# jp-schneider/awesome

Hardware: AMD Instinct MI355X
Metric: INR-fits/sec (256x256 grid, convexity prior) (higher is better)
Workload: dtype f32; 1 GPU; 1 x 256x256 synthetic convex blob per GPU, ConvexNextNet(h=130,L=1), SE(sigmoid) mean, Adam lr 2e-3, clamp, E=2000 full-batch steps (BASELINE configs[1]); images_per_gpu=1, grid=256x256, epochs_per_fit=2000, parallelism=dp1 (independent fits)

## Files before the change

### awesome_amd/csrc/icnn_step.h

```cpp
#pragma once
#include <hip/hip_runtime.h>
#include <stdint.h>
#include <math.h>

#include <type_traits>

#include "inrfit.h"

typedef float f32x4 __attribute__((ext_vector_type(4)));
typedef float f32x2 __attribute__((ext_vector_type(2)));

#define MFMA16(a, b, c) __builtin_amdgcn_mfma_f32_16x16x4f32((a), (b), (c), 0, 0, 0)
__device__ __forceinline__ float relu0(float x) { return __int_as_float(max(__float_as_int(x), 0)); }
constexpr float INV_2PI = 0.15915494309189535f;
__device__ __forceinline__ float hw_sin(float x) { return __builtin_amdgcn_sinf(__builtin_amdgcn_fractf(x * INV_2PI)); }
__device__ __forceinline__ float hw_cos(float x) { return __builtin_amdgcn_cosf(__builtin_amdgcn_fractf(x * INV_2PI)); }
template <int ACT>
__device__ __forceinline__ float act0_f(float pre, float omega) {
    if constexpr (ACT == INR_ACT_COS) return hw_cos(pre);
    else if constexpr (ACT == INR_ACT_SIN) return hw_sin(omega * pre);
    else return relu0(pre);
}
template <int ACT>
__device__ __forceinline__ float dact0_f(float pre, float omega) {
// ... 78 lines not shown
                        : SL_WO + (j - P_WO);
    }
};

struct ImgMap {
    int H, C, L, HM, S, PT, floats;
    int off_sc, off_wine, off_win, off_bin, off_floor, off_wo;
    int off_wct[2], off_w[2];
    int ext[4];
    int p_bin, p_wo, p_bo, p_so, P;
    int p_w[2], p_b[2], p_s[2];
    int sl_tile;
    int sl_cols;
    int KG, kg_magic;
    int identity;
};

__device__ __forceinline__ int slab_param_of_col(const ImgMap& m, int col) {
    if (m.identity) return col < m.sl_cols ? col : -1;
    const int H = m.H, HM = m.HM, C = m.C, KG = m.KG, kgm = m.kg_magic, T = m.sl_tile, two = m.L > 1;
    const int e0 = m.ext[0], e1 = m.ext[1], e2 = m.ext[2], e3 = m.ext[3], pwo = m.p_wo, ncols = m.sl_cols;
    const int tl = (two && col >= T) ? 1 : 0, ct = col - tl * T;
    const int pw = tl ? m.p_w[1] : m.p_w[0], pb = tl ? m.p_b[1] : m.p_b[0], ps = tl ? m.p_s[1] : m.p_s[0];
    const int r = ct & 3, lane = (ct >> 2) & 63, tb = ct >> 8;
    const int rt = (tb * kgm) >> 16, b = tb - rt * KG;
    const int o = 16 * rt + 4 * (lane >> 4) + r, pos = 16 * b + (lane & 15);
    int tile = -1;
    tile = (pos == e3 && C > 2) ? ps + o * C + 2 : tile;
    tile = (pos == e2 && C > 1) ? ps + o * C + 1 : tile;
    tile = pos == e1 ? ps + o * C : tile;
    tile = pos == e0 ? pb + o : tile;
    tile = pos < H ? pw + o * H + pos : tile;
    const int HR = H - HM, LS = HR * (H + 1 + C), NT = two ? 2 * T : T;
    const int c = col - NT, c1 = c - m.p_w[0];
    const int rl = (two && c1 >= LS) ? 1 : 0, cl = c1 - rl * LS;
    const int qw = rl ? m.p_w[1] : m.p_w[0], qb = rl ? m.p_b[1] : m.p_b[0], qs = rl ? m.p_s[1] : m.p_s[0];
    const int c2 = cl - HR * H, c3 = c2 - HR;
    int rest = qs + HM * C + c3;
    rest = c3 < 0 ? qb + HM + c2 : rest;
    rest = c2 < 0 ? qw + HM * H + cl : rest;
    const int ct2 = c1 - (two ? 2 * LS : LS);
    rest = ct2 >= 0 ? pwo + ct2 : rest;
    rest = c1 < 0 ? c : rest;
    const int res = col < NT ? tile : rest;
    return col < ncols ? res : -1;
}

__device__ __forceinline__ int image_slots(const ImgMap& m, int j, int (&slot)[2]) {
    if (j < m.p_bin) {
        const int i = j / m.C, c = j - i * m.C;
        slot[0] = m.off_wine + c * m.PT + i;
        if (i >= m.HM) {
            slot[1] = m.off_win + c * 16 + (i - m.HM);
            return 2;
        }
        return 1;
    }
    if (j < m.p_w[0]) {
        const int i = j - m.p_bin;
        slot[0] = m.off_wine + m.C * m.PT + i;
        if (i >= m.HM) {
            slot[1] = m.off_bin + (i - m.HM);
            return 2;
        }
        return 1;
    }
    for (int k = 0; k < m.L; ++k) {
        if (j < m.p_b[k]) {
            const int q = j - m.p_w[k];
            const int o = q / m.H, i = q - o * m.H;
            slot[0] = m.off_w[k] + o * m.S + i;
            if (i >= m.HM) {
                slot[1] = m.off_wct[k] + (i - m.HM) * m.PT + o;
                return 2;
            }
            return 1;
        }
        if (j < m.p_s[k]) {
            slot[0] = m.off_w[k] + (j - m.p_b[k]) * m.S + m.ext[0];
            return 1;
        }
        if (j < m.p_s[k] + m.H * m.C) {
            const int q = j - m.p_s[k];
            const int o = q / m.C, c = q - o * m.C;
            slot[0] = m.off_w[k] + o * m.S + m.ext[1 + c];
            return 1;
        }
    }
    if (j < m.p_bo) {
        slot[0] = m.off_wo + (j - m.p_wo);
        return 1;
    }
    slot[0] = m.off_sc + (j - m.p_bo);
    return 1;
}

struct StepArgs {
    const float* wimg;
    const float* targets;
    const float* coef;
    float* slabs;
    float* loss_part;
    float* logits;
    float* dcoords;
    InrGridDesc grid;
    long long N;
    int n_images, wgs, PS, loss_kind;
    float act_omega;
    const float* seg;
    float c_align;
    int data_count;
    int use_noneclass;
    float noneclass;
    int align_soft;
    int align_begin;
};

template <int CTRL>
__device__ __forceinline__ float dpp_f(float v) {
    return __int_as_float(__builtin_amdgcn_update_dpp(0, __float_as_int(v), CTRL, 0xF, 0xF, true));
}
__device__ __forceinline__ float bce_log(float x) {
    const float l = logf(x);
    return l < -100.f ? -100.f : l;
}

__device__ __forceinline__ void align_term(const float* __restrict__ seg, float c_align, int soft, float pr, float& l, float& dy) {
    const float s = *seg;
    const float d = pr - (soft ? s : (s > 0.5f ? 1.f : 0.f));
    const float cd = c_align * d;
    l = fmaf(cd, d, l);
    dy = fmaf(2.f * cd, pr * (1.f - pr), dy);
}

__device__ __forceinline__ float sum_over_points(float v) {
    v += dpp_f<0xB1>(v);
    v += dpp_f<0x4E>(v);
    v += dpp_f<0x141>(v);
    v += dpp_f<0x140>(v);
    return v;
}
__device__ __forceinline__ float sum_over_groups(float v) {
    {
        const auto r = __builtin_amdgcn_permlane16_swap(__float_as_uint(v), __float_as_uint(v), false, false);
        v = __uint_as_float(r[0]) + __uint_as_float(r[1]);
    }
    {
        const auto r = __builtin_amdgcn_permlane32_swap(__float_as_uint(v), __float_as_uint(v), false, false);
        v = __uint_as_float(r[0]) + __uint_as_float(r[1]);
    }
    return v;
}

#ifndef INR_SCHED_HINTS
#define INR_SCHED_HINTS 1
#endif
#if INR_SCHED_HINTS
#define SGB(mask, n) __builtin_amdgcn_sched_group_barrier((mask), (n), 0)
#else
#define SGB(mask, n)
#endif
#ifndef INR_BWD_B128
#define INR_BWD_B128 0
#endif
#ifndef INR_STAGE_Z0_EARLY
#define INR_STAGE_Z0_EARLY 1
#endif
#ifndef INR_PROLOGUE_EARLY
#define INR_PROLOGUE_EARLY 1
#endif
#ifndef INR_SLAB_NT
#define INR_SLAB_NT 1
#endif
#ifndef INR_TILES_SPREAD
#define INR_TILES_SPREAD 1
#endif
#ifndef INR_MFMA_ORDER
#define INR_MFMA_ORDER 1
#endif
#if INR_MFMA_ORDER
#define MFMA_STEP_FENCE() __builtin_amdgcn_sched_barrier(0x7F6)
#define OPERAND_FENCE() __builtin_amdgcn_sched_barrier(0x676)
#else
#define MFMA_STEP_FENCE()
#define OPERAND_FENCE()
#endif

#ifndef INR_STAMPS
#define INR_STAMPS 0
#endif
#if INR_STAMPS
__device__ unsigned long long g_stamps[16];
__device__ unsigned long long g_wgtimes[1024][4];
__device__ unsigned long long g_wgfirst[1024];
#define STAMP(k)                                                                                   \
    do {                                                                                           \
        __builtin_amdgcn_sched_barrier(0);                                                         \
        unsigned long long t_;                                                                     \
        asm volatile("s_memtime %0\n\ts_waitcnt lgkmcnt(0)" : "=s"(t_)::"memory");                 \
        __builtin_amdgcn_sched_barrier(0);                                                         \
        st_sum[k] += t_ - st_prev;                                                                 \
        st_prev = t_;                                                                              \
    } while (0)
#else
#define STAMP(k)
#endif

template <int FLOATS>
__device__ __forceinline__ f32x4 image_to_lds_issue(const float* __restrict__ gimg, float* smem, const int tid, const int lane, const int wave) {
    constexpr int PIECES = FLOATS / 256, TAIL4 = (FLOATS - 256 * PIECES) / 4;
    static_assert(FLOATS % 4 == 0 && TAIL4 <= 256, "the tail is one float4 per thread at most");
    f32x4 tail = f32x4{0.f, 0.f, 0.f, 0.f};
    if (tid < TAIL4) tail = ((const f32x4*)gimg)[64 * PIECES + tid];
#pragma unroll
    for (int k = 0; k < (PIECES + 3) / 4; ++k) {
        const int pc = wave + 4 * k;
        if (pc < PIECES)
            __builtin_amdgcn_global_load_lds((const __attribute__((address_space(1))) void*)(gimg + pc * 256 + lane * 4),
                                             (__attribute__((address_space(3))) void*)(smem + pc * 256), 16, 0, 0);
    }
    return tail;
}
template <int FLOATS>
__device__ __forceinline__ void image_tail_to_lds(float* smem, const int tid, const f32x4 tail) {
    constexpr int PIECES = FLOATS / 256, TAIL4 = (FLOATS - 256 * PIECES) / 4;
    if (tid < TAIL4) ((f32x4*)smem)[64 * PIECES + tid] = tail;
}

template <int H, int C, bool TRAIN, bool DX = false, int ACT0 = INR_ACT_RELU>
__global__ __launch_bounds__(WG_THREADS, 1) void icnn_step_kernel(const StepArgs a) {
    static_assert(!DX || TRAIN, "coordinate gradients are a by-product of the backward pass");
    static_assert(!DX || ACT0 == INR_ACT_RELU, "the coordinate-gradient kernels are built for relu networks only");
    using G = Cfg<H, C>;
    constexpr int TM = G::TM, KG = G::KG, HM = G::HM, HR = G::HR, S = G::S, PT = G::PT, RPW = G::RPW, NEXT = G::NEXT;
    constexpr bool B128 = INR_BWD_B128 && (TM % 4 == 0);
    auto bcol = [](int t, int l) { return B128 ? 64 * (t >> 2) + 4 * l + (t & 3) : 16 * t + l; };
    constexpr int HRA = HR > 0 ? HR : 1;
    static_assert(TM % RPW == 0, "row tiles must split evenly over the waves that own rows");
    extern __shared__ __attribute__((aligned(16))) float smem[];
    float* const Wimg = smem + G::OFF_W;
    float* const WcT = smem + G::OFF_WCT;
    float* const WinE = smem + G::OFF_WINE;
    float* const WinT = smem + G::OFF_WIN;
    float* const binT = smem + G::OFF_BIN;
    float* const floorT = smem + G::OFF_FLOOR;
    float* const woT = smem + G::OFF_WO;
    float* const stA = smem + G::OFF_STA;
    float* const stB = smem + G::OFF_STB;

#if INR_STAMPS
    const unsigned long long rt_entry = __builtin_amdgcn_s_memrealtime();
#endif
    const int tid = threadIdx.x;
    const int lane = tid & 63;
    const int wave = __builtin_amdgcn_readfirstlane(tid >> 6);
    const int l15 = lane & 15, g = lane >> 4;
    const int img = blockIdx.x / a.wgs;
    const int wg = blockIdx.x - img * a.wgs;
    const long long N = a.N;

    const float* __restrict__ gimg = a.wimg + (size_t)img * G::IMG_FLOATS;
#if INR_PROLOGUE_EARLY
    static_assert(WG_THREADS == 256, "image_to_lds_issue");
    const f32x4 img_tail = image_to_lds_issue<G::IMG_FLOATS>(gimg, smem, tid, lane, wave);
    __builtin_amdgcn_sched_barrier(0);
#else
    {
        const f32x4* __restrict__ src = (const f32x4*)gimg;
        constexpr int NV4 = G::IMG_FLOATS / 4;
        constexpr int NIT = (NV4 + WG_THREADS - 1) / WG_THREADS;
        f32x4 tmp[NIT];
#pragma unroll
        for (int k = 0; k < NIT; ++k) {
            const int i = tid + k * WG_THREADS;
            if (i < NV4) tmp[k] = src[i];
        }
#pragma unroll
        for (int k = 0; k < NIT; ++k) {
            const int i = tid + k * WG_THREADS;
            if (i < NV4) ((f32x4*)smem)[i] = tmp[k];
        }
    }
#endif
    float cfg_ = 0.f, cbg_ = 0.f;
    if (TRAIN) {
        cfg_ = a.coef[2 * img];
        cbg_ = a.coef[2 * img + 1];
    }
    float b_o, s_o[C];
    float wol[HRA];
    auto image_arrived = [&]() {
        __syncthreads();
        b_o = smem[G::OFF_SC];
#pragma unroll
        for (int c = 0; c < C; ++c) s_o[c] = smem[G::OFF_SC + 1 + c];
#pragma unroll
        for (int u = 0; u < HRA; ++u) wol[u] = HR > 0 ? woT[HM + u] : 0.f;
    };
#if !INR_PROLOGUE_EARLY
    image_arrived();
#endif

    const float* const wf = Wimg + l15 * S + 4 * g;
    const float* const wb = Wimg + l15;
    const bool row_ok = (4 * RPW == TM) || wave * RPW < TM;
    const int arow = 16 * wave * RPW + l15;

    f32x4 dW[RPW][KG];
    constexpr int NQ = (TM + 3) / 4;
    float dL0[NQ][NEXT];
    f32x4 dwo[TM];
    float dwol[HRA];
    float dWl[HRA][KG];
    float dL0l[HRA][NEXT];
    float loss_acc = 0.f, dbo = 0.f, dso[C];
    if (TRAIN) {
#pragma unroll
        for (int j = 0; j < RPW; ++j)
#pragma unroll
            for (int b = 0; b < KG; ++b) dW[j][b] = f32x4{0.f, 0.f, 0.f, 0.f};
#pragma unroll
        for (int t = 0; t < TM; ++t) dwo[t] = f32x4{0.f, 0.f, 0.f, 0.f};
#pragma unroll
        for (int q = 0; q < NQ; ++q)
#pragma unroll
            for (int e = 0; e < NEXT; ++e) dL0[q][e] = 0.f;
#pragma unroll
        for (int u = 0; u < HRA; ++u) {
            dwol[u] = 0.f;
#pragma unroll
            for (int b = 0; b < KG; ++b) dWl[u][b] = 0.f;
#pragma unroll
            for (int e = 0; e < NEXT; ++e) dL0l[u][e] = 0.f;
        }
#pragma unroll
        for (int c = 0; c < C; ++c) dso[c] = 0.f;
    }

    const int n_chunks = (int)((N + SP - 1) / SP);
    struct PointIn {
        float x[C];
        float tg;
    };
    const bool fast_div = N <= (1ll << 24);
    const float inv_width = a.grid.mode == INR_GRID_SEPARABLE ? 1.f / (float)a.grid.width : 0.f;
    auto load_point = [&](int chunk) -> PointIn {
        PointIn q;
        int pc = chunk * SP + wave * 16 + l15;
        pc = pc < (int)N ? pc : (int)N - 1;
        if (a.grid.mode == INR_GRID_SEPARABLE) {
            int row, col;
            if (fast_div) {
                row = (int)((float)pc * inv_width);
                col = pc - row * a.grid.width;
                if (col < 0) {
                    row -= 1;
                    col += a.grid.width;
                } else if (col >= a.grid.width) {
                    row += 1;
                    col -= a.grid.width;
                }
            } else {
                row = pc / a.grid.width;
                col = pc - row * a.grid.width;
            }
            q.x[0] = a.grid.xs[col];
            q.x[1] = a.grid.ys[row];
            if (C > 2) q.x[C - 1] = a.grid.ts ? a.grid.ts[img] : 0.f;
        } else {
            const float* cp = a.grid.coords + (size_t)img * a.grid.coords_image_stride;
#pragma unroll
            for (int c = 0; c < C; ++c) q.x[c] = cp[(size_t)c * N + pc];
        }
        q.tg = TRAIN ? a.targets[(size_t)img * a.data_count + min(pc, a.data_count - 1)] : 0.f;
        return q;
    };
    PointIn nxt = load_point(wg);
#if INR_PROLOGUE_EARLY
    __builtin_amdgcn_sched_barrier(0);
    image_tail_to_lds<G::IMG_FLOATS>(smem, tid, img_tail);
    image_arrived();
    __builtin_amdgcn_sched_barrier(0);
#endif
#if INR_STAMPS
    unsigned long long st_sum[12] = {0, 0, 0, 0, 0, 0, 0, 0, 0, 0, 0, 0}, st_prev;
    asm volatile("s_memtime %0\n\ts_waitcnt lgkmcnt(0)" : "=s"(st_prev)::"memory");
    const unsigned long long st_begin = st_prev;
    unsigned long long st_f0 = 0, st_fsum = 0;
    const unsigned long long rt_loop = __builtin_amdgcn_s_memrealtime();
    unsigned long long st_store = 0;
#endif
    for (int chunk = wg; chunk < n_chunks; chunk += a.wgs) {
#if INR_STAMPS
        if (chunk == wg) {
            __builtin_amdgcn_sched_barrier(0);
            __builtin_amdgcn_s_waitcnt(0);
            if (tid == 0 && blockIdx.x < 1024) g_wgfirst[blockIdx.x] = __builtin_amdgcn_s_memrealtime() - rt_entry;
            __builtin_amdgcn_sched_barrier(0);
        }
#endif
        STAMP(0);
        const int p = chunk * SP + wave * 16 + l15;
        const bool valid = p < (int)N;
        const PointIn cur = nxt;
        float x[C];
#pragma unroll
        for (int c = 0; c < C; ++c) x[c] = cur.x[c];
        const float tg = cur.tg;

        f32x4 z0[KG];
        const float xe = g < C ? x[g < C ? g : 0] : (g == C ? 1.f : 0.f);
        auto z0_tile = [&](int tk) -> f32x4 {
            f32x4 z = MFMA16(WinE[g * PT + 16 * tk + l15], xe, (f32x4{0.f, 0.f, 0.f, 0.f}));
#pragma unroll
            for (int r = 0; r < 4; ++r) z[r] = act0_f<ACT0>(z[r], a.act_omega);
            return z;
        };
        f32x4 z0lpre;
        {
            const int q = 4 * g;
            f32x4 v = *(const f32x4*)&binT[q];
#pragma unroll
            for (int c = 0; c < C; ++c) v += *(const f32x4*)&WinT[c * 16 + q] * x[c];
            const f32x4 fl = *(const f32x4*)&floorT[q];
            z0lpre = v;
#pragma unroll
            for (int r = 0; r < 4; ++r) {
                if constexpr (ACT0 == INR_ACT_RELU) {
                    z0[TM][r] = fmaxf(v[r], fl[r]);
                } else {
                    const bool hid = g == 0 && r < HR;
                    z0[TM][r] = hid ? act0_f<ACT0>(v[r], a.act_omega) : (fl[r] < 0.f ? v[r] : 0.f);
                }
            }
        }

        STAMP(1);
        f32x4 acc[TM];
        float la[HRA];
#pragma unroll
        for (int u = 0; u < HRA; ++u) la[u] = 0.f;
        f32x4 wq[2][TM];
        f32x4 wlq[2][HRA];
        float winq[2];
        f32x4 wo[TM];
#pragma unroll
        for (int t = 0; t < TM; ++t) wq[0][t] = *(const f32x4*)(wf + t * 16 * S);
#pragma unroll
        for (int u = 0; u < HR; ++u) wlq[0][u] = *(const f32x4*)(Wimg + (HM + u) * S + 4 * g);
        z0[0] = z0_tile(0);
        winq[1] = WinE[g * PT + 16 * (TM > 1 ? 1 : 0) + l15];
#pragma unroll
        for (int tk = 0; tk < KG; ++tk) {
            const int cur = tk & 1, nx = cur ^ 1;
            constexpr int NRD = TM + HR + 1;
            auto next_read = [&](int i) {
                if (tk + 1 < KG) {
                    if (i < TM) wq[nx][i] = *(const f32x4*)(wf + i * 16 * S + 16 * (tk + 1));
                    else if (i < TM + HR) wlq[nx][i - TM] = *(const f32x4*)(Wimg + (HM + i - TM) * S + 16 * (tk + 1) + 4 * g);
                    else if (i == TM + HR && tk + 2 < TM) winq[cur] = WinE[g * PT + 16 * (tk + 2) + l15];
                } else if (i < TM) {
                    wo[i] = *(const f32x4*)&woT[16 * i + 4 * g];
                }
            };
#if INR_STAMPS
            if (tk == 2) { __builtin_amdgcn_sched_barrier(0); asm volatile("s_memtime %0\n\ts_waitcnt lgkmcnt(0)" : "=s"(st_f0)::"memory"); __builtin_amdgcn_sched_barrier(0); }
            if (tk == 7) { __builtin_amdgcn_sched_barrier(0); unsigned long long t_; asm volatile("s_memtime %0\n\ts_waitcnt lgkmcnt(0)" : "=s"(t_)::"memory"); __builtin_amdgcn_sched_barrier(0); st_fsum += t_ - st_f0; }
#endif
            if (tk == (KG > 2 ? 1 : 0)) {
                const int cn = chunk + a.wgs;
                nxt = load_point(cn < n_chunks ? cn : chunk);
            }
            f32x4 zn = f32x4{0.f, 0.f, 0.f, 0.f};
            if (tk + 1 < TM) zn = MFMA16(winq[nx], xe, (f32x4{0.f, 0.f, 0.f, 0.f}));
            const int nmf = G::nr_in(tk) * TM;
            const int every = nmf / NRD > 0 ? nmf / NRD : 1;
#pragma unroll
            for (int r = 0; r < G::nr_in(tk); ++r) {
#pragma unroll
                for (int t = 0; t < TM; ++t) {
                    acc[t] = MFMA16(wq[cur][t][r], z0[tk][r], (tk == 0 && r == 0) ? (f32x4{0.f, 0.f, 0.f, 0.f}) : acc[t]);
                    const int q = r * TM + t;
                    if (q % every == every - 1 && q / every < NRD) next_read(q / every);
                    OPERAND_FENCE();
                }
            }
#pragma unroll
            for (int i = 0; i < NRD; ++i)
                if (i >= nmf / every) next_read(i);
#pragma unroll
            for (int u = 0; u < HR; ++u)
#pragma unroll
                for (int r = 0; r < G::nr_in(tk); ++r) la[u] = fmaf(wlq[cur][u][r], z0[tk][r], la[u]);
            if (tk + 1 < TM) {
#pragma unroll
                for (int r = 0; r < 4; ++r) z0[tk + 1][r] = act0_f<ACT0>(zn[r], a.act_omega);
            }
#if INR_STAGE_Z0_EARLY
            if (TRAIN && tk < TM) *(f32x4*)(stB + (wave * 16 + l15) * G::SB + 4 * g + 16 * tk) = z0[tk];
#endif
            __builtin_amdgcn_sched_barrier(0);
        }

        STAMP(2);
        f32x4 z0p[TM];
        if (TRAIN) {
            float wie[TM];
#pragma unroll
            for (int t = 0; t < TM; ++t) wie[t] = WinE[g * PT + bcol(t, l15)];
            OPERAND_FENCE();
#pragma unroll
            for (int t = 0; t < TM; ++t) z0p[t] = MFMA16(xe, wie[t], (f32x4{0.f, 0.f, 0.f, 0.f}));
            MFMA_STEP_FENCE();
        }
        float ypart = 0.f;
#pragma unroll
        for (int t = 0; t < TM; ++t) {
#pragma unroll
            for (int r = 0; r < 4; ++r) {
#if !(defined(INR_EXP_NOVALU) && (INR_EXP_NOVALU & 1))
                acc[t][r] = relu0(acc[t][r]);
#endif
                ypart = fmaf(wo[t][r], acc[t][r], ypart);
            }
        }
        ypart = sum_over_groups(ypart);
        float z1l[HRA];
#pragma unroll
        for (int u = 0; u < HR; ++u) {
            z1l[u] = relu0(sum_over_groups(la[u]));
            ypart = fmaf(wol[u], z1l[u], ypart);
        }
        float y = ypart + b_o;
#pragma unroll
        for (int c = 0; c < C; ++c) y = fmaf(s_o[c], x[c], y);
        if (a.logits != nullptr && valid && g == 0) a.logits[(size_t)img * N + p] = y;

        if (TRAIN) {
            const float pr = 1.f / (1.f + expf(-y));
            const float cw = tg < 0.5f ? cfg_ : cbg_;
            float l, dy;
            if (a.loss_kind == INR_LOSS_SE) {
                const float d = tg - pr;
                l = d * d * cw;
                dy = 2.f * (pr - tg) * pr * (1.f - pr) * cw;
            } else if (a.loss_kind == INR_LOSS_EXTERNAL) {
                l = 0.f;
                dy = tg;
            } else {
                const float lp = bce_log(pr), lq = bce_log(1.f - pr);
// ... 135 lines not shown
                        else dz0[t][r] *= dact0_f<ACT0>(z0p[t][r], a.act_omega);
#endif
                    }
                auto swap32 = [](float& u, float& v) {
                    const auto s = __builtin_amdgcn_permlane32_swap(__float_as_uint(u), __float_as_uint(v), false, false);
                    u = __uint_as_float(s[0]);
                    v = __uint_as_float(s[1]);
                };
                auto swap16 = [](float& u, float& v) {
                    const auto s = __builtin_amdgcn_permlane16_swap(__float_as_uint(u), __float_as_uint(v), false, false);
                    u = __uint_as_float(s[0]);
                    v = __uint_as_float(s[1]);
                };
                const float* const xrow = stB + wave * 16 * G::SB;
#pragma unroll
                for (int r = 0; r < 4; ++r) {
                    float D[NQ][4];
#pragma unroll
                    for (int q = 0; q < NQ; ++q) {
#pragma unroll
                        for (int j = 0; j < 4; ++j) D[q][j] = 4 * q + j < TM ? dz0[4 * q + j < TM ? 4 * q + j : 0][r] : 0.f;
                        swap32(D[q][0], D[q][2]);
                        swap32(D[q][1], D[q][3]);
                        swap16(D[q][0], D[q][1]);
                        swap16(D[q][2], D[q][3]);
                    }
#pragma unroll
                    for (int k = 0; k < 4; ++k) {
                        float xp[C];
#pragma unroll
                        for (int c = 0; c < C; ++c) xp[c] = xrow[(4 * k + r) * G::SB + G::ext_pos(1 + c)];
#pragma unroll
                        for (int q = 0; q < NQ; ++q) {
                            dL0[q][0] += D[q][k];
#pragma unroll
                            for (int c = 0; c < C; ++c) dL0[q][1 + c] = fmaf(D[q][k], xp[c], dL0[q][1 + c]);
                        }
                    }
                }
            }
            float hx[C];
#pragma unroll
            for (int c = 0; c < C; ++c) hx[c] = s_o[c] * dy;
#pragma unroll
            for (int u = 0; u < HR; ++u) {
                const float d = sum_over_groups(dz0l[u]);
                const float z0u = DX ? __shfl(z0[TM][u], l15) : z0[TM][u];
                float dm;
                if constexpr (ACT0 == INR_ACT_RELU) dm = z0u > 0.f ? d : 0.f;
                else dm = d * dact0_f<ACT0>(z0lpre[u], a.act_omega);
                if (DX) {
#pragma unroll
                    for (int c = 0; c < C; ++c) hx[c] = fmaf(WinT[c * 16 + u], dm, hx[c]);
                }
                if (g == 0) {
                    dL0l[u][0] += dm;
#pragma unroll
                    for (int c = 0; c < C; ++c) dL0l[u][1 + c] = fmaf(dm, x[c], dL0l[u][1 + c]);
                }
            }
            if (DX) {
                float part[4][C];
#pragma unroll
                for (int r = 0; r < 4; ++r)
#pragma unroll
                    for (int c = 0; c < C; ++c) part[r][c] = (l15 == G::ext_pos(1 + c) - HM) ? dzx[r] : 0.f;
#pragma unroll
                for (int t = 0; t < TM; ++t)
#pragma unroll
                    for (int c = 0; c < C; ++c) {
                        const float w = WinE[c * PT + bcol(t, l15)];
#pragma unroll
                        for (int r = 0; r < 4; ++r) part[r][c] = fmaf(w, dz0[t][r], part[r][c]);
                    }
                float dxv[C];
#pragma unroll
                for (int c = 0; c < C; ++c) dxv[c] = 0.f;
#pragma unroll
                for (int r = 0; r < 4; ++r)
#pragma unroll
                    for (int c = 0; c < C; ++c) {
                        const float v = sum_over_points(part[r][c]);
                        dxv[c] = l15 == r ? v : dxv[c];
                    }
                const int pp = chunk * SP + wave * 16 + 4 * g + l15;
#pragma unroll
                for (int c = 0; c < C; ++c) {
                    const float v = dxv[c] + __shfl(hx[c], 4 * g + l15);
                    if (l15 < 4 && pp < (int)N) a.dcoords[((size_t)img * C + c) * N + pp] = v;
                }
            }
            STAMP(5);
            __syncthreads();
            STAMP(6);

            {
                auto stage_pt = [&](int it) { const int s = (it + wave) & 15; return 16 * (s >> 2) + (s & 3) + 4 * g; };
                float af[2][RPW], bf[2][KG];
                {
                    const int pt = stage_pt(0);
#pragma unroll
                    for (int j = 0; j < RPW; ++j) af[0][j] = stA[pt * G::SA + arow + 16 * j];
#pragma unroll
                    for (int b = 0; b < KG; ++b) bf[0][b] = stB[pt * G::SB + 16 * b + l15];
                }
#pragma unroll
                for (int it = 0; it < SP / 4; ++it) {
                    const int cur = it & 1, nx = cur ^ 1;
                    const int ptc = stage_pt(it), ptn = stage_pt(it + 1 < SP / 4 ? it + 1 : it);
                    auto next_read = [&](int i) {
                        if (it + 1 < SP / 4) {
                            if (i < RPW) af[nx][i] = stA[ptn * G::SA + arow + 16 * i];
                            else if (i < RPW + KG) bf[nx][i - RPW] = stB[ptn * G::SB + 16 * (i - RPW) + l15];
                        }
                    };
                    if (HR > 0 && (it & 3) == 0) {
                        const f32x4 dl = *(const f32x4*)(stA + ptc * G::SA + HM);
#pragma unroll
                        for (int u = 0; u < HR; ++u)
#pragma unroll
                            for (int b = 0; b < KG; ++b) dWl[u][b] = fmaf(dl[u], bf[cur][b], dWl[u][b]);
                    }
                    if (row_ok) {
#pragma unroll
                        for (int j = 0; j < RPW; ++j)
#pragma unroll
                            for (int b = 0; b < KG; ++b) {
                                dW[j][b] = MFMA16(af[cur][j], bf[cur][b], dW[j][b]);
                                next_read(j * KG + b);
                                OPERAND_FENCE();
                            }
                    } else {
#pragma unroll
                        for (int i = 0; i < RPW + KG; ++i) next_read(i);
                    }
                    if (RPW * KG < RPW + KG) {
#pragma unroll
                        for (int i = RPW * KG; i < RPW + KG; ++i) next_read(i);
                    }
                    __builtin_amdgcn_sched_barrier(0);
                }
            }
            STAMP(7);
            __syncthreads();
            STAMP(8);
        }
    }
#if INR_STAMPS
    unsigned long long st_loop_end;
    asm volatile("s_memtime %0\n\ts_waitcnt lgkmcnt(0)" : "=s"(st_loop_end)::"memory");
    const unsigned long long rt_loop_end = __builtin_amdgcn_s_memrealtime();
#endif

    if (TRAIN) {
        float* __restrict__ slab = a.slabs + ((size_t)img * a.wgs + wg) * a.PS;
        constexpr int NTILES = RPW * KG, UW = 4 * TM + HR * KG;
#if !INR_TILES_SPREAD
        {
            constexpr int tile_from = 0, tile_to = NTILES;
#include "icnn_step_tiles.h"
        }
#endif
        constexpr int SC_DWO = 0;
        constexpr int SC_DWL = SC_DWO + PT;
        constexpr int SC_L0L = SC_DWL + HRA * PT;
        constexpr int SC_SC = SC_L0L + HRA * 4;
        constexpr int SC_L0 = SC_SC + 8;
        constexpr int WSTR = SC_L0 + HM * 4;
        static_assert(4 * WSTR <= SP * G::SA, "reduction scratch must fit stage A");
        float* const scr = stA + wave * WSTR;
#pragma unroll
        for (int t = 0; t < TM; ++t) {
#pragma unroll
            for (int r = 0; r < 4; ++r) {
                const float v = sum_over_points(dwo[t][r]);
                if (l15 == 0) scr[SC_DWO + 16 * t + 4 * g + r] = v;
            }
#if INR_TILES_SPREAD
            {
                const int tile_from = 4 * t * NTILES / UW, tile_to = (4 * t + 4) * NTILES / UW;
#include "icnn_step_tiles.h"
            }
#endif
        }
#pragma unroll
        for (int u = 0; u < HR; ++u) {
            const float v = sum_over_points(dwol[u]);
            if (lane == 0) scr[SC_DWO + HM + u] = v;
#pragma unroll
            for (int b = 0; b < KG; ++b) {
                const float w = sum_over_groups(dWl[u][b]);
                if (g == 0) scr[SC_DWL + u * PT + 16 * b + l15] = w;
#if INR_TILES_SPREAD
                {
                    const int tile_from = (4 * TM + u * KG + b) * NTILES / UW, tile_to = (4 * TM + u * KG + b + 1) * NTILES / UW;
#include "icnn_step_tiles.h"
                }
#endif
            }
#pragma unroll
            for (int e = 0; e < NEXT; ++e) {
                const float w = sum_over_points(dL0l[u][e]);
                if (lane == 0) scr[SC_L0L + u * 4 + e] = w;
            }
        }
#pragma unroll
        for (int q = 0; q < NQ; ++q)
            if (4 * q + g < TM) {
#pragma unroll
                for (int e = 0; e < NEXT; ++e) scr[SC_L0 + bcol(4 * q + g, l15) * 4 + e] = dL0[q][e];
            }
        {
            float sc[2 + C];
            sc[0] = loss_acc;
            sc[1] = dbo;
#pragma unroll
            for (int c = 0; c < C; ++c) sc[2 + c] = dso[c];
#pragma unroll
            for (int k = 0; k < 2 + C; ++k) {
                const float v = sum_over_points(sc[k]);
                if (lane == 0) scr[SC_SC + k] = v;
            }
        }
        __syncthreads();
        auto wsum = [&](int i) { return ((stA[i] + stA[WSTR + i]) + stA[2 * WSTR + i]) + stA[3 * WSTR + i]; };
        for (int i = tid; i < H; i += WG_THREADS) slab[G::SL_WO + i] = wsum(SC_DWO + i);
        for (int i = tid; i < HR * PT; i += WG_THREADS) {
            const int u = i / PT, pos = i - u * PT;
            const float v = wsum(SC_DWL + i);
            if (pos < H) slab[G::SL_W1L + u * H + pos] = v;
            else if (pos == G::ext_pos(0)) slab[G::SL_B1L + u] = v;
            else {
#pragma unroll
                for (int c = 0; c < C; ++c)
                    if (pos == G::ext_pos(1 + c)) slab[G::SL_S1L + u * C + c] = v;
            }
        }
        for (int i = tid; i < HM * NEXT; i += WG_THREADS) {
            const int row = i / NEXT, e = i - row * NEXT;
            const float v = wsum(SC_L0 + row * 4 + e);
            if (e == 0) slab[G::SL_TILE + G::P_BIN + row] = v;
            else slab[G::SL_TILE + G::P_WIN + row * C + (e - 1)] = v;
        }
        if (tid < HR * NEXT) {
            const int u = tid / NEXT, e = tid - u * NEXT;
            const float v = wsum(SC_L0L + u * 4 + e);
            if (e == 0) slab[G::SL_TILE + G::P_BIN + HM + u] = v;
            else slab[G::SL_TILE + G::P_WIN + (HM + u) * C + (e - 1)] = v;
        }
        if (tid < 2 + C) {
            const float v = wsum(SC_SC + tid);
            if (tid == 0) {
                slab[G::SL_LOSS] = v;
                a.loss_part[(size_t)img * a.wgs + wg] = v;
            } else if (tid == 1) slab[G::slab_col(G::P_BO)] = v;
            else slab[G::slab_col(G::P_SO) + tid - 2] = v;
        }
    }
#if INR_STAMPS
    unsigned long long st_wait = 0;
    if (TRAIN) {
        __builtin_amdgcn_sched_barrier(0);
        asm volatile("s_memtime %0\n\ts_waitcnt lgkmcnt(0)" : "=s"(st_wait)::"memory");
        __builtin_amdgcn_sched_barrier(0);
    }
    if (TRAIN && (tid & 63) == 0 && blockIdx.x < 1024) {
        __builtin_amdgcn_s_waitcnt(0);
        const unsigned long long rt_end = __builtin_amdgcn_s_memrealtime();
        if (tid == 0) {
            g_wgtimes[blockIdx.x][0] = rt_entry;
            g_wgtimes[blockIdx.x][1] = rt_loop;
            g_wgtimes[blockIdx.x][2] = rt_loop_end;
        }
        atomicMax(&g_wgtimes[blockIdx.x][3], rt_end);
    }
    if (TRAIN && blockIdx.x == 0 && tid == 0) {
        unsigned long long t_end;
        asm volatile("s_memtime %0\n\ts_waitcnt lgkmcnt(0)" : "=s"(t_end)::"memory");
        for (int k = 0; k < 9; ++k) g_stamps[k] = st_sum[k];
        g_stamps[9] = st_begin;
        g_stamps[10] = st_loop_end - st_begin;
        g_stamps[11] = t_end - st_loop_end;
        g_stamps[12] = st_fsum;
        g_stamps[13] = t_end - st_store;
        g_stamps[14] = t_end - st_wait;
    }
#endif
}

}
```

### awesome_amd/csrc/inrfit.hip

```cpp
#include "icnn_step.h"
#include "icnn_step2.h"
#include "flow.h"
#include "rnvp.h"
#include "joint_loss.h"
#include "wide.h"
#include "star.h"
#include "cnnseg.h"
#include "fcseg.h"

#include <type_traits>
#include <vector>

namespace {

constexpr int UPD_RANGES = WIDE_MAX_LAYERS + 1;
struct UpdArgs {
    float* wimg;
    ImgMap img;
    float* params;
    float* opt_state;
    const float* slabs;
    const float* loss_part;
    long long loss_stride;
    float* loss_hist;
// ... 2940 lines not shown
    return joint_prior_step_run(FusedIcnn(), model, params, opt_state, grid, seg, target, desc, seg_term, opt, step, loss_out, dseg,
                                prior_logits, status, workspace, workspace_bytes, (hipStream_t)stream);
}

int inrfit_wide_joint_prior_step(const InrModelDesc* model, float* params, float* opt_state, const InrGridDesc* grid, const float* seg,
                                 const float* target, const InrJointPriorDesc* desc, const float* seg_term, const InrOptDesc* opt,
                                 int step, float* loss_out, float* dseg, float* prior_logits, int32_t* status, void* workspace,
                                 int64_t workspace_bytes, void* stream) {
    return joint_prior_step_run(WideIcnn(), model, params, opt_state, grid, seg, target, desc, seg_term, opt, step, loss_out, dseg,
                                prior_logits, status, workspace, workspace_bytes, (hipStream_t)stream);
}

static int check_star(const InrStarDesc* star, int64_t n_points, void* workspace, int64_t workspace_bytes, StarMap* m, StarWs* w) {
    if (!star || star->n_hidden < 1 || star->n_hidden > STAR_MAX_HIDDEN) return INR_EUNSUPPORTED;
    if (n_points <= 0 || n_points * (int64_t)star->n_hidden > (int64_t)1 << 31) return INR_EINVAL;
    if (!workspace) return INR_EINVAL;
    *m = make_star_map(star->n_hidden);
    *w = carve_star(star->n_hidden, n_points, workspace);
    if (workspace_bytes < w->bytes) return INR_EWORKSPACE;
    return INR_OK;
}

int64_t inrfit_star_param_count(const InrStarDesc* star) {
    if (!star || star->n_hidden < 1 || star->n_hidden > STAR_MAX_HIDDEN) return INR_EUNSUPPORTED;
    return make_star_map(star->n_hidden).P;
}

int64_t inrfit_star_workspace_bytes(const InrStarDesc* star, int64_t n_points) {
    if (!star || star->n_hidden < 1 || star->n_hidden > STAR_MAX_HIDDEN) return INR_EUNSUPPORTED;
    if (n_points <= 0 || n_points * (int64_t)star->n_hidden > (int64_t)1 << 31) return INR_EINVAL;
    return carve_star(star->n_hidden, n_points, nullptr).bytes;
}

int inrfit_star_forward(const InrStarDesc* star, const float* params, const float* coords, int64_t n_points, float* logits,
                        void* workspace, int64_t workspace_bytes, void* stream) {
    StarMap m;
    StarWs w;
    if (!params || !coords || !logits) return INR_EINVAL;
    int rc = check_star(star, n_points, workspace, workspace_bytes, &m, &w);
    if (rc) return rc;
    hipStream_t s = (hipStream_t)stream;
    if ((rc = star_forward_pass(m, w, params, coords, nullptr, n_points, n_points, nullptr, logits, s))) return rc;
    return hipGetLastError() == hipSuccess ? INR_OK : INR_ELAUNCH;
}

static void star_upd_consts(StarUpdArgs& u, const InrOptDesc* opt, int t, int t_off) {
    u.lr = opt->lr;
    u.beta1 = opt->beta1;
    u.beta2 = opt->beta2;
    u.eps = opt->eps;
    u.one_minus_b1 = (float)(1.0 - (double)opt->beta1);
    u.one_minus_b2 = (float)(1.0 - (double)opt->beta2);
    bias_corrections(opt, t, &u.bc1, &u.bc2_sqrt);
    u.offset_on = t_off > 0;
    u.bc1_off = 1.0;
    u.bc2_sqrt_off = 1.f;
    if (t_off > 0) bias_corrections(opt, t_off, &u.bc1_off, &u.bc2_sqrt_off);
}

int inrfit_star_loss_grad(const InrStarDesc* star, const float* params, const float* coords, const float* labels, int64_t n_pixels,
                          const int32_t* index, int64_t batch, float* loss, float* grads, void* workspace, int64_t workspace_bytes,
                          void* stream) {
    StarMap m;
    StarWs w;
    if (!params || !coords || !labels || !grads || n_pixels <= 0 || batch > STAR_MAX_BATCH) return INR_EINVAL;
    if (!index && batch > n_pixels) return INR_EINVAL;
    int rc = check_star(star, batch, workspace, workspace_bytes, &m, &w);
    if (rc) return rc;
    hipStream_t s = (hipStream_t)stream;
    if ((rc = star_forward_pass(m, w, params, coords, index, n_pixels, batch, labels, nullptr, s))) return rc;
    if ((rc = star_backward_pass(m, w, params, batch, loss, 0, s))) return rc;
    StarUpdArgs u{};
    u.prm = nullptr;
    u.gW1 = w.gW1;
    u.colp = w.colp;
    u.scal = w.scal;
    u.grads_out = grads;
    u.m = m;
    u.mode = 1;
    hipLaunchKernelGGL(star_update_kernel, dim3((m.P + 255) / 256), dim3(256), 0, s, u);
    return hipGetLastError() == hipSuccess ? INR_OK : INR_ELAUNCH;
}

int inrfit_star_fit(const InrStarDesc* star, float* params, float* opt_state, const float* coords, const float* labels,
                    int64_t n_pixels, const int32_t* batch_index, int64_t batch, const InrOptDesc* opt, int32_t steps, int32_t step0,
                    int32_t offset_first_step, float* loss_hist, void* workspace, int64_t workspace_bytes, void* stream) {
    StarMap m;
    StarWs w;
    if (!params || !opt_state || !coords || !labels || !batch_index || !opt || steps < 0 || step0 < 0 || n_pixels <= 0) return INR_EINVAL;
    if (opt->kind != INR_OPT_ADAM || batch > STAR_MAX_BATCH) return INR_EINVAL;
    int rc = check_star(star, batch, workspace, workspace_bytes, &m, &w);
    if (rc) return rc;
    hipStream_t s = (hipStream_t)stream;
    StarUpdArgs u{};
    u.prm = params;
    u.opt = opt_state;
    u.gW1 = w.gW1;
    u.colp = w.colp;
    u.scal = w.scal;
    u.m = m;
    u.mode = 0;
    for (int it = 0; it < steps; ++it) {
        const int ep = step0 + it;
        const int32_t* idx = batch_index + (size_t)it * batch;
        if ((rc = star_forward_pass(m, w, params, coords, idx, n_pixels, batch, labels, nullptr, s))) return rc;
        if ((rc = star_backward_pass(m, w, params, batch, loss_hist, it, s))) return rc;
        star_upd_consts(u, opt, ep + 1, offset_first_step >= 0 && ep >= offset_first_step ? ep - offset_first_step + 1 : 0);
        hipLaunchKernelGGL(star_update_kernel, dim3((m.P + 255) / 256), dim3(256), 0, s, u);
    }
    return hipGetLastError() == hipSuccess ? INR_OK : INR_ELAUNCH;
}

__global__ __launch_bounds__(256) void debug_tanh_exp_kernel(const float* __restrict__ x, long long n, float* __restrict__ th,
                                                              float* __restrict__ ex) {
    const long long i = (long long)blockIdx.x * 256 + threadIdx.x;
    if (i < n) {
        th[i] = fast_tanh(x[i]);
        ex[i] = fast_exp(x[i]);
    }
}

int inrfit_debug_tanh_exp(const float* x, int64_t n, float* tanh_out, float* exp_out, void* stream) {
    if (!x || !tanh_out || !exp_out || n <= 0) return INR_EINVAL;
    hipLaunchKernelGGL(debug_tanh_exp_kernel, dim3((unsigned)((n + 255) / 256)), dim3(256), 0, (hipStream_t)stream, x, (long long)n,
                       tanh_out, exp_out);
    return hipGetLastError() == hipSuccess ? INR_OK : INR_ELAUNCH;
}

int inrfit_miou(const float* out, const float* tgt, int n_images, int64_t n_points, float thr_out, float thr_tgt, int invert,
                float* iou, void* stream) {
    if (!out || !tgt || !iou || n_images <= 0 || n_points <= 0) return INR_EINVAL;
    hipLaunchKernelGGL(miou_kernel, dim3(n_images), dim3(256), 0, (hipStream_t)stream, out, tgt, (long long)n_points, thr_out,
                       thr_tgt, invert, iou);
    return hipGetLastError() == hipSuccess ? INR_OK : INR_ELAUNCH;
}

int inrfit_pack_masks(const float* values, int n_images, int64_t n_points, float threshold, int invert, uint64_t* bits,
                      void* stream) {
    if (!values || !bits || n_images <= 0 || n_points <= 0) return INR_EINVAL;
    const long long words = (n_points + 63) / 64;
    hipLaunchKernelGGL(pack_masks_kernel, dim3((unsigned)((words + 3) / 4), n_images), dim3(256), 0, (hipStream_t)stream, values,
                       (long long)n_points, threshold, invert, (unsigned long long*)bits);
    return hipGetLastError() == hipSuccess ? INR_OK : INR_ELAUNCH;
}

#if INR_STAMPS
int inrfit_debug_updtimes(unsigned long long* host_out) {
    return hipMemcpyFromSymbol(host_out, HIP_SYMBOL(g_updtimes), sizeof(unsigned long long) * 2048) == hipSuccess ? 0 : -4;
}
int inrfit_debug_updissue(unsigned long long* host_out) {
    return hipMemcpyFromSymbol(host_out, HIP_SYMBOL(g_updissue), sizeof(unsigned long long) * 512) == hipSuccess ? 0 : -4;
}
int inrfit_debug_wgfirst(unsigned long long* host_out) {
    return hipMemcpyFromSymbol(host_out, HIP_SYMBOL(g_wgfirst), sizeof(unsigned long long) * 1024) == hipSuccess ? 0 : -4;
}
int inrfit_debug_stamps2(unsigned long long* host_out) {
    return hipMemcpyFromSymbol(host_out, HIP_SYMBOL(g_stamps2), sizeof(unsigned long long) * 16) == hipSuccess ? 0 : -4;
}
int inrfit_debug_stamps(unsigned long long* host_out) {
    return hipMemcpyFromSymbol(host_out, HIP_SYMBOL(g_stamps), sizeof(unsigned long long) * 16) == hipSuccess ? 0 : -4;
}
int inrfit_debug_wgtimes(unsigned long long* host_out) {
    if (hipMemcpyFromSymbol(host_out, HIP_SYMBOL(g_wgtimes), sizeof(unsigned long long) * 4096) != hipSuccess) return -4;
    static unsigned long long zeros[4096];
    return hipMemcpyToSymbol(HIP_SYMBOL(g_wgtimes), zeros, sizeof(zeros)) == hipSuccess ? 0 : -4;
}
#endif

const char* inrfit_strerror(int code) {
    switch (code) {
        case INR_OK: return "ok";
        case INR_EINVAL: return "invalid argument";
        case INR_EUNSUPPORTED: return "model shape has no compiled kernel";
        case INR_EWORKSPACE: return "workspace too small";
        case INR_ELAUNCH: return "HIP launch failed";
        case INR_ENODEVICE: return "no gfx950 device";
        default: return "unknown error";
    }
}

}


namespace {

struct FcWs {
    int P, blocks;
    long long count;
    float *slab, *loss;
    long long bytes;
};

static bool fc_desc_ok(const InrFcSegDesc* d) {
    return d && d->width == FC_WIDTH && d->depth >= 0 && d->depth <= FC_MAX_DEPTH && d->in_channels >= 1 && d->in_channels <= FC_MAX_IN &&
           d->image_channels >= 0 && d->image_channels <= d->in_channels && d->n_rows >= 1 && d->n_rows < (1LL << 40) &&
           d->data_count >= 0 && d->data_count <= d->n_rows;
}

static long long fc_param_count(const InrFcSegDesc* d) {
    return (long long)fc_b_off(d->in_channels, d->depth, d->depth + 1) + 1;
}

static FcWs fc_layout(const InrFcSegDesc* d, void* base) {
    FcWs w{};
    w.P = (int)fc_param_count(d);
    const long long chunks = (d->n_rows + FC_BLOCK - 1) / FC_BLOCK;
    w.blocks = (int)(chunks < FC_MAX_BLOCKS ? chunks : FC_MAX_BLOCKS);
    w.count = d->data_count > 0 ? d->data_count : d->n_rows;
    w.slab = (float*)base;
    const long long slab_bytes = ((long long)w.blocks * (w.P + 1) * 4 + 255) / 256 * 256;
    w.loss = (float*)((char*)base + slab_bytes);
    w.bytes = slab_bytes + 256;
    return w;
}

static int fc_check(const InrFcSegDesc* d, const float* const* wts, const float* const* bs, const float* image, const float* feat,
                    void* ws, long long ws_bytes, FcWs* w) {
    if (!d || !wts || !bs || !ws) return INR_EINVAL;
    if (!fc_desc_ok(d)) return INR_EUNSUPPORTED;
    if ((d->image_channels > 0 && !image) || (d->image_channels < d->in_channels && !feat)) return INR_EINVAL;
    for (int l = 0; l < d->depth + 2; ++l)
        if (!wts[l] || !bs[l]) return INR_EINVAL;
    *w = fc_layout(d, ws);
    if (ws_bytes < w->bytes) return INR_EWORKSPACE;
    return INR_OK;
}

template <bool BWD>
static void fc_launch_rows(int depth, int blocks, hipStream_t s, const FcArgs& a) {
    const dim3 grid(blocks), block(FC_BLOCK);
    switch (depth) {
        case 0: hipLaunchKernelGGL((fc_rows_kernel<0, BWD>), grid, block, 0, s, a); break;
        case 1: hipLaunchKernelGGL((fc_rows_kernel<1, BWD>), grid, block, 0, s, a); break;
        case 2: hipLaunchKernelGGL((fc_rows_kernel<2, BWD>), grid, block, 0, s, a); break;
        default: hipLaunchKernelGGL((fc_rows_kernel<3, BWD>), grid, block, 0, s, a); break;
    }
}

static FcArgs fc_args(const FcWs& w, const InrFcSegDesc* d, const float* const* wts, const float* const* bs, const float* image,
                      const float* feat, const float* target, const float* dseg, float* logits, float* seg) {
    FcArgs a{};
    for (int l = 0; l < d->depth + 2; ++l) {
        a.w[l] = wts[l];
        a.b[l] = bs[l];
    }
    a.image = image;
    a.feat = feat;
    a.target = target;
    a.dseg = dseg;
    a.logits = logits;
    a.seg = seg;
    a.slab = w.slab;
    a.n = d->n_rows;
    a.count = w.count;
    a.F = d->in_channels;
    a.ic = d->image_channels;
    a.inversion = d->inversion;
    a.P = w.P;
    a.seed_scale = (float)((double)d->g / (double)w.count);
    return a;
}

}

extern "C" {

int64_t inrfit_fcseg_param_count(const InrFcSegDesc* desc) {
    InrFcSegDesc d;
    if (!desc) return -1;
    d = *desc;
    if (d.n_rows < 1) d.n_rows = 1;
    if (d.data_count < 0 || d.data_count > d.n_rows) d.data_count = 0;
    return fc_desc_ok(&d) ? fc_param_count(&d) : -1;
}

int64_t inrfit_fcseg_workspace_bytes(const InrFcSegDesc* desc) { return fc_desc_ok(desc) ? fc_layout(desc, nullptr).bytes : -1; }

int inrfit_fcseg_forward(const InrFcSegDesc* desc, const float* const* weights, const float* const* biases, const float* image_rows,
                         const float* feature_rows, const float* target, float* logits, float* seg, float* loss_out, void* workspace,
                         int64_t workspace_bytes, void* stream) {
    FcWs w;
    int rc = fc_check(desc, weights, biases, image_rows, feature_rows, workspace, workspace_bytes, &w);
    if (rc) return rc;
    if (target && !loss_out) return INR_EINVAL;
    hipStream_t s = (hipStream_t)stream;
    FcArgs a = fc_args(w, desc, weights, biases, image_rows, feature_rows, target, nullptr, logits, seg);
    a.P = 0;
    a.stride = 1;
    fc_launch_rows<false>(desc->depth, w.blocks, s, a);
    if (target) {
        FcReduceArgs r{w.slab, w.blocks, 1, 0, desc->g, (float)w.count, nullptr, nullptr, loss_out, w.loss};
        hipLaunchKernelGGL(fc_reduce_kernel, dim3(1), dim3(FC_REDUCE_BLOCK), 0, s, r);
    }
    return hipGetLastError() == hipSuccess ? INR_OK : INR_ELAUNCH;
}

int inrfit_fcseg_step(const InrFcSegDesc* desc, const float* const* weights, const float* const* biases, const float* image_rows,
                      const float* feature_rows, const float* target, const float* dseg, int reuse_forward, float* logits, float* seg,
                      float* loss_out, float* grads, int32_t* status, void* workspace, int64_t workspace_bytes, void* stream) {
    FcWs w;
    int rc = fc_check(desc, weights, biases, image_rows, feature_rows, workspace, workspace_bytes, &w);
    if (rc) return rc;
    if (!target || !grads || !status) return INR_EINVAL;
    (void)reuse_forward;
    hipStream_t s = (hipStream_t)stream;
    FcArgs a = fc_args(w, desc, weights, biases, image_rows, feature_rows, target, dseg, logits, seg);
    a.stride = w.P + 1;
// ... 8 lines not shown
```

Measured before the change: 6.988 fits/s.

## Defer image wait into loop, batch image DMA, level-batched cross-lane reductions

Moves the wait for the image to arrive in LDS into the first loop iteration, so point loading and setup overlap the image transfer. Issues the per-wave image DMA pieces in contiguous runs using immediate offsets instead of strided pieces. Replaces the final per-value wave reductions with reductions that run level by level across many values at once, staging per-wave partials in LDS and summing the four waves in one pass. This adds more code paths and LDS scratch, and the offset-based DMA addressing is harder to verify.

```diff
diff --git a/awesome_amd/csrc/icnn_step.h b/awesome_amd/csrc/icnn_step.h
--- a/awesome_amd/csrc/icnn_step.h
+++ b/awesome_amd/csrc/icnn_step.h
@@ -254,6 +254,31 @@
     return v;
 }
 
+template <int NV>
+__device__ __forceinline__ void sum_over_points_by_level(float (&v)[NV]) {
+#pragma unroll
+    for (int i = 0; i < NV; ++i) v[i] += dpp_f<0xB1>(v[i]);
+#pragma unroll
+    for (int i = 0; i < NV; ++i) v[i] += dpp_f<0x4E>(v[i]);
+#pragma unroll
+    for (int i = 0; i < NV; ++i) v[i] += dpp_f<0x141>(v[i]);
+#pragma unroll
+    for (int i = 0; i < NV; ++i) v[i] += dpp_f<0x140>(v[i]);
+}
+template <int NV>
+__device__ __forceinline__ void sum_over_groups_by_level(float (&v)[NV]) {
+#pragma unroll
+    for (int i = 0; i < NV; ++i) {
+        const auto r = __builtin_amdgcn_permlane16_swap(__float_as_uint(v[i]), __float_as_uint(v[i]), false, false);
+        v[i] = __uint_as_float(r[0]) + __uint_as_float(r[1]);
+    }
+#pragma unroll
+    for (int i = 0; i < NV; ++i) {
+        const auto r = __builtin_amdgcn_permlane32_swap(__float_as_uint(v[i]), __float_as_uint(v[i]), false, false);
+        v[i] = __uint_as_float(r[0]) + __uint_as_float(r[1]);
+    }
+}
+
 #ifndef INR_SCHED_HINTS
 #define INR_SCHED_HINTS 1
 #endif
@@ -276,6 +301,15 @@
 #endif
 #ifndef INR_TILES_SPREAD
 #define INR_TILES_SPREAD 1
+#endif
+#ifndef INR_IMAGE_WAIT_IN_LOOP
+#define INR_IMAGE_WAIT_IN_LOOP 1
+#endif
+#ifndef INR_IMAGE_DMA_RUNS
+#define INR_IMAGE_DMA_RUNS 1
+#endif
+#ifndef INR_SUMS_BY_LEVEL
+#define INR_SUMS_BY_LEVEL 1
 #endif
 #ifndef INR_MFMA_ORDER
 #define INR_MFMA_ORDER 1
@@ -294,7 +328,7 @@
 #if INR_STAMPS
 __device__ unsigned long long g_stamps[16];
 __device__ unsigned long long g_wgtimes[1024][4];
-__device__ unsigned long long g_wgfirst[1024];
+__device__ unsigned long long g_wgfirst[2][1024];
 #define STAMP(k)                                                                                   \
     do {                                                                                           \
         __builtin_amdgcn_sched_barrier(0);                                                         \
@@ -314,6 +348,22 @@
     static_assert(FLOATS % 4 == 0 && TAIL4 <= 256, "the tail is one float4 per thread at most");
     f32x4 tail = f32x4{0.f, 0.f, 0.f, 0.f};
     if (tid < TAIL4) tail = ((const f32x4*)gimg)[64 * PIECES + tid];
+#if INR_IMAGE_DMA_RUNS
+    constexpr int PPW = (PIECES + 3) / 4;
+    const int p0 = wave * PPW;
+#define INR_DMA_PIECE(j)                                                                                                           \
+    if (k + (j) < PPW && (3 * PPW + k + (j) < PIECES || p0 + k + (j) < PIECES))                                                    \
+        __builtin_amdgcn_global_load_lds((const __attribute__((address_space(1))) void*)(gimg + (p0 + k) * 256 + lane * 4),          \
+                                         (__attribute__((address_space(3))) void*)(smem + (p0 + k) * 256), 16, 1024 * (j), 0)
+#pragma unroll
+    for (int k = 0; k < PPW; k += 4) {
+        INR_DMA_PIECE(0);
+        INR_DMA_PIECE(1);
+        INR_DMA_PIECE(2);
+        INR_DMA_PIECE(3);
+    }
+#undef INR_DMA_PIECE
+#else
 #pragma unroll
     for (int k = 0; k < (PIECES + 3) / 4; ++k) {
         const int pc = wave + 4 * k;
@@ -321,6 +371,7 @@
             __builtin_amdgcn_global_load_lds((const __attribute__((address_space(1))) void*)(gimg + pc * 256 + lane * 4),
                                              (__attribute__((address_space(3))) void*)(smem + pc * 256), 16, 0, 0);
     }
+#endif
     return tail;
 }
 template <int FLOATS>
@@ -402,6 +453,7 @@
 #if !INR_PROLOGUE_EARLY
     image_arrived();
 #endif
+    constexpr bool WAIT_IN_LOOP = INR_PROLOGUE_EARLY && INR_IMAGE_WAIT_IN_LOOP;
 
     const float* const wf = Wimg + l15 * S + 4 * g;
     const float* const wb = Wimg + l15;
@@ -478,11 +530,18 @@
         return q;
     };
     PointIn nxt = load_point(wg);
-#if INR_PROLOGUE_EARLY
+#if INR_STAMPS
+    unsigned long long rt_image = rt_entry;
+#endif
+#if INR_PROLOGUE_EARLY && !INR_IMAGE_WAIT_IN_LOOP
     __builtin_amdgcn_sched_barrier(0);
     image_tail_to_lds<G::IMG_FLOATS>(smem, tid, img_tail);
     image_arrived();
     __builtin_amdgcn_sched_barrier(0);
+#if INR_STAMPS
+    rt_image = __builtin_amdgcn_s_memrealtime();
+    __builtin_amdgcn_sched_barrier(0);
+#endif
 #endif
 #if INR_STAMPS
     unsigned long long st_sum[12] = {0, 0, 0, 0, 0, 0, 0, 0, 0, 0, 0, 0}, st_prev;
@@ -493,11 +552,27 @@
     unsigned long long st_store = 0;
 #endif
     for (int chunk = wg; chunk < n_chunks; chunk += a.wgs) {
+#if INR_PROLOGUE_EARLY && INR_IMAGE_WAIT_IN_LOOP
+        if (chunk == wg) {
+            __builtin_amdgcn_sched_barrier(0);
+            image_tail_to_lds<G::IMG_FLOATS>(smem, tid, img_tail);
+            image_arrived();
+            __builtin_amdgcn_sched_barrier(0);
+#if INR_STAMPS
+            rt_image = __builtin_amdgcn_s_memrealtime();
+            __builtin_amdgcn_sched_barrier(0);
+#endif
+        }
+#endif
 #if INR_STAMPS
         if (chunk == wg) {
             __builtin_amdgcn_sched_barrier(0);
             __builtin_amdgcn_s_waitcnt(0);
-            if (tid == 0 && blockIdx.x < 1024) g_wgfirst[blockIdx.x] = __builtin_amdgcn_s_memrealtime() - rt_entry;
+            if (tid == 0 && blockIdx.x < 1024) {
+                const unsigned long long rt_first = __builtin_amdgcn_s_memrealtime();
+                g_wgfirst[0][blockIdx.x] = rt_first - rt_entry;
+                g_wgfirst[1][blockIdx.x] = rt_first - rt_image;
+            }
             __builtin_amdgcn_sched_barrier(0);
         }
 #endif
@@ -939,6 +1014,10 @@
     const unsigned long long rt_loop_end = __builtin_amdgcn_s_memrealtime();
 #endif
 
+    if (WAIT_IN_LOOP && wg >= n_chunks) {
+        image_tail_to_lds<G::IMG_FLOATS>(smem, tid, img_tail);
+        __syncthreads();
+    }
     if (TRAIN) {
         float* __restrict__ slab = a.slabs + ((size_t)img * a.wgs + wg) * a.PS;
         constexpr int NTILES = RPW * KG, UW = 4 * TM + HR * KG;
@@ -948,6 +1027,115 @@
 #include "icnn_step_tiles.h"
         }
 #endif
+#if INR_SUMS_BY_LEVEL
+        constexpr int NREST = G::SL_COLS - G::SL_TILE;
+        constexpr int SC_WIN = G::P_WIN, SC_BIN = G::P_BIN, SC_W1L = G::SL_W1L - G::SL_TILE, SC_B1L = G::SL_B1L - G::SL_TILE;
+        constexpr int SC_S1L = G::SL_S1L - G::SL_TILE, SC_WO = G::SL_WO - G::SL_TILE;
+        constexpr int SC_DUMP = round_up(NREST, 4);
+        constexpr int WSTR = SC_DUMP + 64;
+        static_assert(4 * WSTR <= SP * G::SA, "reduction scratch must fit stage A");
+        static_assert(G::SL_LOSS == G::SL_COLS - 1 && G::slab_col(G::P_BO) == G::SL_WO + H, "the scalars follow w_o, the loss column is the last");
+        float* const scr = stA + wave * WSTR;
+        const int dump = SC_DUMP + lane;
+        {
+            const int r3 = l15 & 3;
+            float* const scr_wo = scr + SC_WO + 4 * g + r3;
+#pragma unroll
+            for (int t = 0; t < TM; ++t) {
+                float v[4];
+#pragma unroll
+                for (int r = 0; r < 4; ++r) v[r] = dwo[t][r];
+                sum_over_points_by_level(v);
+                float own = v[0];
+#pragma unroll
+                for (int r = 1; r < 4; ++r) own = r3 == r ? v[r] : own;
+                scr_wo[16 * t] = own;
+#if INR_TILES_SPREAD
+                {
+                    const int tile_from = 4 * t * NTILES / UW, tile_to = (4 * t + 4) * NTILES / UW;
+#include "icnn_step_tiles.h"
+                }
+#endif
+            }
+        }
+#pragma unroll
+        for (int u = 0; u < HR; ++u) {
+            int last = dump;
+            last = l15 < HR ? SC_W1L + u * H + HM + l15 : last;
+            last = HM + l15 == G::ext_pos(0) ? SC_B1L + u : last;
+#pragma unroll
+            for (int c = 0; c < C; ++c) last = HM + l15 == G::ext_pos(1 + c) ? SC_S1L + u * C + c : last;
+#pragma unroll
+            for (int k = 0; k < (KG + 3) / 4; ++k) {
+                constexpr int NB = 4;
+                float w[NB];
+#pragma unroll
+                for (int j = 0; j < NB; ++j) w[j] = 4 * k + j < KG ? dWl[u][4 * k + j < KG ? 4 * k + j : 0] : 0.f;
+                sum_over_groups_by_level(w);
+                float own = w[0];
+#pragma unroll
+                for (int j = 1; j < NB; ++j) own = g == j ? w[j] : own;
+                const int b = 4 * k + g;
+                const int adr = b < TM ? SC_W1L + u * H + 16 * b + l15 : (b == TM ? last : dump);
+                scr[adr] = own;
+#if INR_TILES_SPREAD
+                {
+                    const int unit = 4 * TM + u * KG, b_to = 4 * k + 4 < KG ? 4 * k + 4 : KG;
+                    const int tile_from = (unit + 4 * k) * NTILES / UW, tile_to = (unit + b_to) * NTILES / UW;
+#include "icnn_step_tiles.h"
+                }
+#endif
+            }
+        }
+#pragma unroll
+        for (int q = 0; q < NQ; ++q)
+            if (4 * q + g < TM) {
+                const int unit = bcol(4 * q + g, l15);
+                scr[SC_BIN + unit] = dL0[q][0];
+#pragma unroll
+                for (int c = 0; c < C; ++c) scr[SC_WIN + unit * C + c] = dL0[q][1 + c];
+            }
+        {
+            constexpr int N1 = HR + C + 2, N2 = HR, N3 = HR * C, NS = N1 + N2 + N3;
+            float sv[NS];
+#pragma unroll
+            for (int u = 0; u < HR; ++u) {
+                sv[u] = dwol[u];
+                sv[N1 + u] = dL0l[u][0];
+#pragma unroll
+                for (int c = 0; c < C; ++c) sv[N1 + N2 + u * C + c] = dL0l[u][1 + c];
+            }
+            sv[HR] = dbo;
+#pragma unroll
+            for (int c = 0; c < C; ++c) sv[HR + 1 + c] = dso[c];
+            sv[HR + 1 + C] = loss_acc;
+            sum_over_points_by_level(sv);
+#pragma unroll
+            for (int w = 0; w < (NS + 15) / 16; ++w) {
+                float own = sv[16 * w];
+#pragma unroll
+                for (int j = 1; j < 16; ++j)
+                    if (16 * w + j < NS) own = l15 == j ? sv[16 * w + j < NS ? 16 * w + j : 0] : own;
+                const int idx = 16 * w + l15;
+                int adr = dump;
+                adr = idx < NS ? SC_WIN + HM * C + (idx - N1 - N2) : adr;
+                adr = idx < N1 + N2 ? SC_BIN + HM + (idx - N1) : adr;
+                adr = idx < N1 ? SC_WO + HM + idx : adr;
+                adr = g == 0 ? adr : dump;
+                scr[adr] = own;
+            }
+        }
+        __syncthreads();
+#pragma unroll
+        for (int i0 = 0; i0 < NREST; i0 += WG_THREADS) {
+            const int i = i0 + tid;
+            if (i < NREST) {
+                const float v = ((stA[i] + stA[WSTR + i]) + stA[2 * WSTR + i]) + stA[3 * WSTR + i];
+                slab[G::SL_TILE + i] = v;
+                if (i == NREST - 1) a.loss_part[(size_t)img * a.wgs + wg] = v;
+            }
+        }
+#else
         constexpr int SC_DWO = 0;
         constexpr int SC_DWL = SC_DWO + PT;
         constexpr int SC_L0L = SC_DWL + HRA * PT;
@@ -1043,6 +1231,7 @@
             } else if (tid == 1) slab[G::slab_col(G::P_BO)] = v;
             else slab[G::slab_col(G::P_SO) + tid - 2] = v;
         }
+#endif
     }
 #if INR_STAMPS
     unsigned long long st_wait = 0;
diff --git a/awesome_amd/csrc/inrfit.hip b/awesome_amd/csrc/inrfit.hip
--- a/awesome_amd/csrc/inrfit.hip
+++ b/awesome_amd/csrc/inrfit.hip
@@ -3116,7 +3116,7 @@
     return hipMemcpyFromSymbol(host_out, HIP_SYMBOL(g_updissue), sizeof(unsigned long long) * 512) == hipSuccess ? 0 : -4;
 }
 int inrfit_debug_wgfirst(unsigned long long* host_out) {
-    return hipMemcpyFromSymbol(host_out, HIP_SYMBOL(g_wgfirst), sizeof(unsigned long long) * 1024) == hipSuccess ? 0 : -4;
+    return hipMemcpyFromSymbol(host_out, HIP_SYMBOL(g_wgfirst), sizeof(unsigned long long) * 2048) == hipSuccess ? 0 : -4;
 }
 int inrfit_debug_stamps2(unsigned long long* host_out) {
     return hipMemcpyFromSymbol(host_out, HIP_SYMBOL(g_stamps2), sizeof(unsigned long long) * 16) == hipSuccess ? 0 : -4;
```

New measurement: 7.050 fits/s (median of 6 runs). About the same (+0.9%).
